# mbed92/soft-grip

Measured on AMD Instinct MI355X. Metric: env steps/sec (whole node) at batch=4096, higher is better.
Workload: dtype f64; 1 GPU; configs[2]: 4096 envs/GPU, softbox scene (nv=118), stiffness ~ U(300,1400), reference 200-step squeeze schedule from reset, 7 substeps per env step; 327 equality rows (composite neighbour equalities on: DESIGN.md 2, U2); volume tendon damper integrated explicitly; envs_per_gpu=4096, envs_flagged_bad=0

## Files before the change

### soft-grip_amd/csrc/sg_phase.hip

```cpp
#include "sg_work.h"

struct GenLds {
  StageRec2* stage;
  double* gas;
  double* gg;
  double* tmp;
  const double (*boxp)[3];
  const double (*boxm)[9];
  const ChainKin* K;
  const ChainLds2* cs;
  const double *qe, *ve, *asme, *we;
};

__device__ __forceinline__ void sg_gen_capsule(const SgPhaseArgs& a, const GenLds& L, int e, double* cp, double* cax) {
  const int N = a.nelem;
  auto EL = [&](int f, int k) { return a.elem[(size_t)f * N + k]; };
  const double dq = L.qe[e] - EL(SGE_QPOS0, e);
  cp[0] = EL(SGE_GX, e) + EL(SGE_AX, e) * dq; cp[1] = EL(SGE_GY, e) + EL(SGE_AY, e) * dq; cp[2] = EL(SGE_GZ, e) + EL(SGE_AZ, e) * dq;
  cax[0] = EL(SGE_CX, e); cax[1] = EL(SGE_CY, e); cax[2] = EL(SGE_CZ, e);
}

__device__ __noinline__ int sg_gen_phase(const SgPhaseArgs& a, const SgPlanHeader& H, const int env, const GenLds L, int* flags, int* touch) {
  const int lane = threadIdx.x, N = a.nelem;
  auto EL = [&](int f, int k) { return a.elem[(size_t)f * N + k]; };
// ... 656 lines not shown
          for (int r = 0; r < 3; r++) ro[(26 + r) * SG_SPW] = c.f[r];
          ((int*)(ro + 29 * SG_SPW))[0] = sl;
          }
        }
        const int nk = (ns0 > ns1 ? ns0 : ns1) - 32 * k;
        if (a.rowlayout && nk > 0) {
          const int nwb8 = (a.nenv + 7) / 8;
          const int li = lane & 31;
          auto X = [&](int sl_, int L) -> double2* {
            return (double2*)&Sm.stage[sl_ >> 4][32 * k] + ((sl_ & 15) * 8 + L);
          };
          __syncthreads();
          double2* const e0 = (double2*)&Sm.stage[li >> 4][32 * k] + ((li & 15) * 8 + 4 * half);
#pragma unroll
          for (int pr = 0; pr < SG_RK / 2; pr++) {
            e0[0] = fp[0][pr]; e0[1] = fp[1][pr]; e0[2] = fp[2][pr]; e0[3] = fp[3][pr];
            __syncthreads();
#pragma unroll
            for (int j = 0; j < 4; j++) {
              if (8 * j >= nk) break;
              const int e = j * 64 + lane, s_ = e >> 3, L = e & 7;
              if (s_ < nk) *(double2*)(W.crow + SG_ROW_INDEX(32 * k + s_, env >> 3, 2 * pr, 8 * (env & 7) + L, nwb8)) = *X(s_, L);
            }
            __syncthreads();
          }
        }
      }
      SG_T(5);
      double eqR[R], eqb[R], eqf[R];
      double tbp = 0, tjp = 0, tAp = 0;
#pragma unroll
      for (int r = 0; r < R; r++) {
        int e = r * 64 + lane;
        eqR[r] = 1; eqb[r] = 0; eqf[r] = 0;
        if (e < N) {
          double pos = qe[r] - EL(SGE_QPOS0, e), imp = impedance(H.eqj_solimp, pos, 0);
          eqR[r] = fmax(SG_MINVAL, (1 - imp) / imp * EL(SGE_INVW, e));
          double aref = -H.eqj_B * ve[r] - H.eqj_K * imp * pos;
          eqb[r] = asme[r] - aref;
          eqf[r] = -(we[r] - aref) / eqR[r];
          tbp += coef[r] * asme[r]; tjp += coef[r] * we[r]; tAp += coef[r] * coef[r] * invm[r];
        }
      }
      const int nnb = NB ? H.nnb : 0;
      constexpr int ND = NB ? 3 : 0;
      int nbe2[R][3], nbid[R][3];
      double nbc0[R][3];
      [[maybe_unused]] double nbff[R][3];
      [[maybe_unused]] double* const gnbf = W.nbf + (size_t)env * 3 * N;
#pragma unroll
      for (int r = 0; r < R; r++)
#pragma unroll
        for (int d = 0; d < 3; d++) { nbe2[r][d] = -1; nbid[r][d] = -1; nbc0[r][d] = 0; nbff[r][d] = 0; }
      if constexpr (NB) {
        const double im0 = 1.0 / (EL(SGE_MASS, 0) + EL(SGE_ARMATURE, 0));
        const SG_CONSTAS int* const cposc = (const SG_CONSTAS int*)a.cpos;
        const bool wantc = a.rowlayout && a.cst_rounds;
#pragma unroll
        for (int r = 0; r < R; r++) {
          const int e = r * 64 + lane;
          if (e < N) {
            double c4[4] = {0.0, 0.0, 0.0, 0.0};
            if (wantc) c4[0] = sg_div(im0, im0 + eqR[r]);
#pragma unroll
            for (int d = 0; d < 3; d++) {
              const int e2 = nbtabc[d * N + e];
              if (e2 >= 0) {
                const int id = nbtabc[(3 + d) * N + e];
                const double pos = (qe[r] - EL(SGE_QPOS0, e)) - (Sm.as[e2] - EL(SGE_QPOS0, e2)), imp = impedance(H.eqj_solimp, pos, 0);
                const double Rr = fmax(SG_MINVAL, (1 - imp) / imp * (EL(SGE_INVW, e) + EL(SGE_INVW, e2)));
                const double aref = -H.eqj_B * (ve[r] - Sm.ve[e2]) - H.eqj_K * imp * pos;
                const double bb = (asme[r] - Sm.asme[e2]) - aref, ff = -((we[r] - Sm.we[e2]) - aref) / Rr;
                nbe2[r][d] = e2; nbid[r][d] = id; nbc0[r][d] = ff * (0.5 * Rr * ff + bb);
                nbff[r][d] = ff; gnbf[id] = ff;
                W.nbb[(size_t)env * 3 * N + id] = bb; W.nbR[(size_t)env * 3 * N + id] = Rr;
                if (wantc) c4[1 + d] = sg_div(im0, 2.0 * im0 + Rr);
              }
            }
            if (wantc) {
              double* const dst = W.cst + SG_CST_INDEX(env >> 2, 0, 16 * (env & 3), a.cst_rounds) + cposc[e];
              *(double2*)dst = make_double2(c4[0], c4[1]);
              *(double2*)(dst + 2) = make_double2(c4[2], c4[3]);
            }
          }
        }
      }
      const double tpos = L0 - H.t0_L0, timp = impedance(H.eqt_solimp, tpos, 0), tR = fmax(SG_MINVAL, (1 - timp) / timp * H.eqt_invw);
      const double taref = -H.eqt_B * Ld - H.eqt_K * timp * tpos;
      const double tb = wave_sum2(tbp) - taref, tjar = wave_sum2(tjp) - taref, tA = wave_sum2(tAp) + tR;
      double tf = -tjar / tR;
      const int nmaxs = ns0 > ns1 ? ns0 : ns1;

      double aF[SG_CD];
      auto recompute_a = [&]() {
        __syncthreads();
#pragma unroll
        for (int r = 0; r < R; r++) {
          int e = r * 64 + lane;
          if (e < N) {
            double fe = eqf[r] + coef[r] * tf;
            if constexpr (NB) {
#pragma unroll
              for (int d = 0; d < 3; d++) if (nbid[r][d] >= 0) fe += nbff[r][d];
              double fin[3];
#pragma unroll
              for (int d = 0; d < 3; d++) { const int ii = nbtabc[(6 + d) * N + e]; fin[d] = ii >= 0 ? gnbf[ii] : 0.0; }
#pragma unroll
              for (int d = 0; d < 3; d++) fe -= fin[d];
            }
            double as_ = invm[r] * fe;
#pragma unroll
            for (int cb = 0; cb < SG_MAXCH * SG_CG; cb++) {
              const int u = Sm.eslot[e][cb], i0 = u & 0x3F, nst = u >> 6;
              if (nst >= 1) as_ += cval_at(cb / SG_CG, i0);
              if (nst >= 2) as_ += cval_at(cb / SG_CG, i0 + 1);
            }
            if constexpr (GEN)
              if (ngen) as_ += GL.gas[e];
            Sm.as[e] = as_;
          }
        }
        __syncthreads();
        double g[SG_CD] = {0, 0, 0, 0};
#pragma unroll
        for (int k = 0; k < CPL; k++)
#pragma unroll
          for (int d = 0; d < SG_CD; d++) g[d] += cg[k][d];
        if (is_chain_lane) {
          const int la = CS.lim_active;
#pragma unroll
          for (int k = 0; k < SG_MAXLIM; k++)
            if (la >> k & 1) g[k / 2] += CS.lim_sign[k] * CS.lim_f[k];
          if constexpr (GEN)
            if (ngen) {
#pragma unroll
              for (int d = 0; d < SG_CD; d++) g[d] += GL.gg[half * SG_CD + d];
            }
        }
#pragma unroll
        for (int d = 0; d < SG_CD; d++) {
          double x = g[d];
#pragma unroll
          for (int o = 16; o > 0; o >>= 1) x += __shfl_xor(x, o);
          g[d] = x;
        }
#pragma unroll
        for (int a2 = 0; a2 < SG_CD; a2++) {
          double s2 = 0;
#pragma unroll
          for (int b2 = 0; b2 < SG_CD; b2++) s2 += CS.Minv[4 * a2 + b2] * g[b2];
          aF[a2] = s2;
        }
        __syncthreads();
      };
      recompute_a();
      SG_T(6);
      {
        double cp = 0, tJap = 0;
#pragma unroll
        for (int r = 0; r < R; r++) {
          int e = r * 64 + lane;
          if (e < N) {
            double ae = Sm.as[e]; cp += eqf[r] * (0.5 * (ae + eqR[r] * eqf[r]) + eqb[r]); tJap += coef[r] * ae;
#pragma unroll
            for (int d = 0; d < ND; d++)
              if (nbid[r][d] >= 0) cp += 0.5 * nbff[r][d] * (ae - Sm.as[nbe2[r][d]]) + nbc0[r][d];
          }
        }
        double tJa = wave_sum2(tJap);
        if (lane == 0) cp += tf * (0.5 * (tJa + tR * tf) + tb);
        if (is_chain_lane) {
          const int la = CS.lim_active;
#pragma unroll
          for (int k = 0; k < SG_MAXLIM; k++)
            if (la >> k & 1) cp += CS.lim_f[k] * (0.5 * (CS.lim_sign[k] * aF[k / 2] + CS.lim_R[k] * CS.lim_f[k]) + CS.lim_b[k]);
        }
#pragma unroll
        for (int k = 0; k < CPL; k++)
          if ((lane & 31) + 32 * k < myn) {
            double as_ = csl_[k] >= 0 ? Sm.as[csl_[k]] : 0.0, ga = 0;
#pragma unroll
            for (int d = 0; d < SG_CD; d++) ga += cg[k][d] * aF[d];
            cp += 0.5 * (ga + cjsf[k] * as_) + ccost0[k];
          }
        [[maybe_unused]] double aF2[SG_MAXCH][SG_CD];
        if constexpr (GEN)
          if (ngen) {
#pragma unroll
            for (int d = 0; d < SG_CD; d++) {
              const double other = __shfl_xor(aF[d], 32);
              aF2[0][d] = high ? other : aF[d]; aF2[1][d] = high ? aF[d] : other;
            }
            cp += sg_gen_cost(a, env, ngen, aF2, Sm.as, 0);
          }
        double cost = wave_sum2(cp);
        if (cost > 0) {
          if constexpr (GEN)
            if (ngen) {
              sg_gen_cost(a, env, ngen, aF2, Sm.as, 1);
              for (int e = lane; e < N; e += 64) GL.gas[e] = 0.0;
              if (lane < SG_MAXCH * SG_CD) GL.gg[lane] = 0.0;
            }
#pragma unroll
          for (int r = 0; r < R; r++) {
            eqf[r] = 0;
#pragma unroll
            for (int d = 0; d < ND; d++) if (nbid[r][d] >= 0) { nbff[r][d] = 0.0; gnbf[nbid[r][d]] = 0.0; }
          }
          tf = 0;
          if (is_chain_lane) {
#pragma unroll
            for (int k = 0; k < SG_MAXLIM; k++) CS.lim_f[k] = 0;
          }
#pragma unroll
          for (int k = 0; k < CPL; k++) {
            int i = (lane & 31) + 32 * k;
            cjsf[k] = 0;
#pragma unroll
            for (int d = 0; d < SG_CD; d++) cg[k][d] = 0;
            if (i < myn) {
              cval_at(half, i) = 0.0;
              if (!a.rowlayout) {
              double* ro = W.crec + SG_REC_INDEX(i, env / SG_EPW, 0, 2 * (env % SG_EPW) + half, nwb);
#pragma unroll
              for (int r = 0; r < 3; r++) ro[(26 + r) * SG_SPW] = 0.0;
              }
              if (a.rowlayout) {
#pragma unroll
                for (int r = 0; r < 3; r++)
                  *(double2*)(W.crow + SG_ROW_INDEX(i, env >> 3, 6, 8 * (env & 7) + 4 * half + r, (a.nenv + 7) / 8)) = make_double2(0.0, 0.0);
              }
            }
          }
          __syncthreads();
          recompute_a();
        }
      }
      SG_T(7);
#pragma unroll
      for (int r = 0; r < R; r++) {
        int e = r * 64 + lane;
        if (e < N) {
          size_t o = (size_t)env * N + e;
          W.as[o] = Sm.as[e]; W.eqf[o] = eqf[r]; W.eqb[o] = eqb[r]; W.eqR[o] = eqR[r];
        }
      }
      if (is_chain_lane) {
        W.ns[st] = myn < SG_CAP ? myn : SG_CAP;
        W.lim_active[st] = CS.lim_active;
      }
      if (half < nchain) {
        static_assert(4 * SG_MAXLIM == 32, "one limit value per lane of a half");
        const int i = lane & 31;
        W.lim[(size_t)i * S + st] = (&CS.lim_sign[0])[i];
        if (i < SG_CD) W.saF[(size_t)i * S + st] = i == 0 ? aF[0] : (i == 1 ? aF[1] : (i == 2 ? aF[2] : aF[3]));
      }
      if (lane == 0) {
        W.envh[(size_t)0 * a.nenv + env] = tb; W.envh[(size_t)1 * a.nenv + env] = tR;
        W.envh[(size_t)2 * a.nenv + env] = tA; W.envh[(size_t)3 * a.nenv + env] = tf;
        W.shared[env] = shared_slider;
        W.pending[env] = 1;
        W.ncon[env] = ns0 + ns1 + ngen;
        W.gen[env] = ngen;
        W.nefc[env] = N + nnb + 1 + 3 * (ns0 + ns1 + ngen) + __popc(Sm.cs[0].lim_active) + (nchain > 1 ? __popc(Sm.cs[1].lim_active) : 0);
        W.touch[env] = touch;
      }
    }
  }

  SG_T(8);
  __syncthreads();
#pragma unroll
  for (int r = 0; r < R; r++) {
    int e = r * 64 + lane;
    if (e < N) { gq[e0 + e] = qe[r]; gv[e0 + e] = ve[r]; gw[e0 + e] = we[r]; }
  }
  if (lane == 0) {
    if (status | flags) atomicOr(&W.status[env], status | flags);
  }
  SG_T(9);
  SG_TEND();
}

#ifndef SG_X_PHASE_OCC
#define SG_X_PHASE_OCC 2
#endif
#ifndef SG_X_CPL
#define SG_X_CPL 2
#endif
template <int R, int CPL, bool NB, bool GEN = false>
__global__ __launch_bounds__(64, SG_X_PHASE_OCC) void sg_phase_kernel(SgPhaseArgs a) {
  if constexpr (GEN) {
    const int cnt = a.w.gen_count[0];
    a.do_finish = 0; a.do_reset = 0; a.sens = nullptr;
    for (int i = blockIdx.x; i < cnt && i < a.nenv; i += gridDim.x) {
      sg_phase_env<R, CPL, NB, true>(a, a.w.gen_list[i]);
      __syncthreads();
    }
  } else {
    sg_phase_env<R, CPL, NB, false>(a, blockIdx.x);
  }
}

__global__ __launch_bounds__(64) void sg_chain_kernel(SgPhaseArgs a) {
  const int lane = threadIdx.x, c = blockIdx.x & 1, env = (int)(blockIdx.x >> 1) * 64 + lane;
  if (blockIdx.x == 0 && lane == 0) a.w.gen_count[0] = 0;
  SG_T0();
  const SG_CONSTAS SgPlanHeader& H = *(const SG_CONSTAS SgPlanHeader*)a.H;
  const int nv = a.nv, nu = a.nu;
  const size_t S = 2 * (size_t)a.nenv;
  if (env >= a.nenv) return;
  const size_t st = 2 * (size_t)env + c;
  if (a.mask && !a.mask[env]) return;
  SgWork& W = a.w;
  if (a.first && c == 0) { W.status[env] = 0; if (!a.do_finish) W.pending[env] = 0; }
  if (c >= a.nchain) return;
  const int status = a.first ? 0 : W.status[env];
  const int pend = a.do_finish ? W.pending[env] : 0;
  const SgChain& C = H.chain[c];
  const double h = a.timestep;
  double* gq = a.qpos + (size_t)env * nv;
  double* gv = a.qvel + (size_t)env * nv;
  double* gw = a.warm + (size_t)env * nv;
  const double kenv = a.kenv[env];
  double q[SG_CD], v[SG_CD], w[SG_CD], kk[SG_CD], act = 0, ctrl = 0;
#pragma unroll
  for (int d = 0; d < SG_CD; d++) {
    int j = C.dof0 + d;
    if (a.do_reset) { q[d] = C.qpos0[d]; v[d] = 0; w[d] = 0; }
    else { q[d] = gq[j]; v[d] = gv[j]; w[d] = gw[j]; }
    kk[d] = a.kmask_jnt[j] ? kenv : C.stiffness[d];
  }
  if (C.has_act) {
    if (a.do_reset) a.ctrl[(size_t)env * nu + C.act_id] = 0;
    else { act = a.act[(size_t)env * nu + C.act_id]; ctrl = a.ctrl[(size_t)env * nu + C.act_id]; }
  }
  const double kten = C.has_ten ? (a.kmask_ten[C.ten_id] ? kenv : C.ten_k0) : 0.0;
  double* ch = W.chh + st * SG_CHW;
  bool bad_acc = false;
  if (status & (SG_FLAG_BADQPOS | SG_FLAG_BADQVEL | SG_FLAG_BADQACC)) return;

  SG_T(17);
  if (a.do_finish && pend) {
    double aF[SG_CD], qacc_c[SG_CD];
#pragma unroll
    for (int d = 0; d < SG_CD; d++) {
      aF[d] = W.saF[(size_t)d * S + st];
      qacc_c[d] = ch[SGH_QSM + d] + aF[d];
      if (isbad(qacc_c[d])) bad_acc = true;
    }
    ChainKin K;
    {
      double* kd = (double*)&K;
#pragma unroll
      for (int i = 0; i < 48; i++) kd[i] = ch[SGH_K + i];
    }
    if (a.sens) {
      ChainMotion Mo;
      chain_motion(C, K, v, qacc_c, H.gravity, Mo);
      double* so = a.sens + (size_t)env * a.sens_stride;
      for (int s = 0; s < C.nsite; s++) {
        int bi = C.s_body[s];
        double r3[3], sm[9], t[3], t2[3], acc[3], out[3], sbp[3], sbm[9], bw[3], bal[3];
        chain_body_pose(K, bi, sbp, sbm);
        mulmat3(r3, sbm, C.s_pos[s]);
        mulmat33(sm, sbm, C.s_mat[s]);
        for (int k = 0; k < 3; k++) { bw[k] = bi == 0 ? Mo.w[0][k] : Mo.w[SG_CB - 1][k]; bal[k] = bi == 0 ? Mo.al[0][k] : Mo.al[SG_CB - 1][k]; }
        if (C.s_gyro_adr[s] >= 0) {
          mulmatT3(out, sm, bw);
          for (int k = 0; k < 3; k++) so[C.s_gyro_adr[s] + k] = out[k];
        }
        if (C.s_acc_adr[s] >= 0) {
          for (int k = 0; k < 3; k++) acc[k] = bi == 0 ? Mo.a[0][k] : Mo.a[SG_CB - 1][k];
          cross3(t, bal, r3); addscl3(acc, t, 1);
          cross3(t, bw, r3); cross3(t2, bw, t); addscl3(acc, t2, 1);
          mulmatT3(out, sm, acc);
          for (int k = 0; k < 3; k++) so[C.s_acc_adr[s] + k] = out[k];
        }
      }
    }
    if (bad_acc) {
      atomicOr(&W.status[env], SG_FLAG_BADQACC);
    } else {
#pragma unroll
      for (int d = 0; d < SG_CD; d++) w[d] = qacc_c[d];
      if (a.finish_integrate) {
        bool damp = false;
#pragma unroll
        for (int d = 0; d < SG_CD; d++) damp |= C.damping[d] > 0;
        double qa[SG_CD];
        if (damp) {
          double MhB[16], MhBinv[16], rhs[SG_CD], Mm[16];
#pragma unroll
          for (int i = 0; i < 16; i++) { Mm[i] = ch[SGH_M + i]; MhB[i] = Mm[i]; }
#pragma unroll
          for (int d = 0; d < SG_CD; d++) MhB[5 * d] += h * C.damping[d];
          spd_inverse4(MhB, MhBinv);
#pragma unroll
          for (int a2 = 0; a2 < SG_CD; a2++) {
            double s2 = ch[SGH_QFRC + a2];
#pragma unroll
            for (int b2 = 0; b2 < SG_CD; b2++) s2 += Mm[4 * a2 + b2] * aF[b2];
            rhs[a2] = s2;
          }
#pragma unroll
          for (int a2 = 0; a2 < SG_CD; a2++) {
            double s2 = 0;
#pragma unroll
            for (int b2 = 0; b2 < SG_CD; b2++) s2 += MhBinv[4 * a2 + b2] * rhs[b2];
            qa[a2] = s2;
          }
        } else {
#pragma unroll
          for (int d = 0; d < SG_CD; d++) qa[d] = qacc_c[d];
        }
        act += h * ch[SGH_ACTDOT];
#pragma unroll
        for (int d = 0; d < SG_CD; d++) { v[d] += h * qa[d]; q[d] += h * v[d]; }
      }
    }
  }

  SG_T(18);
  if (a.do_begin && !bad_acc) {
    int bad = 0;
#pragma unroll
    for (int d = 0; d < SG_CD; d++) bad |= (isbad(q[d]) ? SG_FLAG_BADQPOS : 0) | (isbad(v[d]) ? SG_FLAG_BADQVEL : 0);
    if (bad) {
      atomicOr(&W.status[env], bad);
    } else {
      ChainKin K;
      ChainDyn D;
      chain_kinematics(C, q, K);
      SG_T(19);
      chain_dynamics(C, K, q, v, act, ctrl, kk, kten, H.gravity, D);
      SG_T(20);
      double rec[SG_CHW];
#pragma unroll
      for (int i = 0; i < SG_CHW; i++) rec[i] = 0.0;
#pragma unroll
      for (int d = 0; d < SG_CD; d++) { rec[SGH_QSM + d] = D.qacc_smooth[d]; rec[SGH_QFRC + d] = D.qfrc_smooth[d]; rec[SGH_V + d] = v[d]; rec[SGH_W + d] = w[d]; }
      rec[SGH_ACTDOT] = D.act_dot;
#pragma unroll
      for (int i = 0; i < 16; i++) { rec[SGH_M + i] = D.M[i]; rec[SGH_MINV + i] = D.Minv[i]; W.sMinv[(size_t)i * S + st] = D.Minv[i]; }
      {
        const double* kd = (const double*)&K;
#pragma unroll
        for (int i = 0; i < 48; i++) rec[SGH_K + i] = kd[i];
      }
#pragma unroll
      for (int g = 0; g < SG_CG; g++) {
        double t[3] = {0, 0, 0}, bp_[3] = {0, 0, 0}, bm_[9], bm2[9];
#pragma unroll
        for (int k = 0; k < 9; k++) bm2[k] = 0;
        if (g < C.ngeom) {
          chain_body_pose(K, C.g_body[g], bp_, bm_);
          mulmat3(t, bm_, C.g_pos[g]);
          mulmat33(bm2, bm_, C.g_mat[g]);
        }
#pragma unroll
        for (int k = 0; k < 3; k++) rec[SGH_BOX + 12 * g + k] = bp_[k] + t[k];
#pragma unroll
        for (int k = 0; k < 9; k++) rec[SGH_BOX + 12 * g + 3 + k] = bm2[k];
      }
      SG_T(21);
      LimitRows L;
      limits_build(C, q, v, D.qacc_smooth, w, L);
      rec[SGH_LIMACT] = (double)L.active;
#pragma unroll
      for (int k = 0; k < SG_MAXLIM; k++) { rec[SGH_LIMSIGN + k] = L.sign[k]; rec[SGH_LIMR + k] = L.R[k]; rec[SGH_LIMB + k] = L.b[k]; rec[SGH_LIMF + k] = L.f[k]; }
      static_assert(SG_CHW % 2 == 0 && SGH_LIMF + SG_MAXLIM <= SG_CHW, "hand-off record layout");
#pragma unroll
      for (int i = 0; i < (SGH_LIMF + SG_MAXLIM + 1) / 2; i++) ((double2*)ch)[i] = make_double2(rec[2 * i], rec[2 * i + 1]);
    }
  }
  SG_T(22);
#pragma unroll
  for (int d = 0; d < SG_CD; d++) { int j = C.dof0 + d; gq[j] = q[d]; gv[j] = v[d]; gw[j] = w[d]; }
  if (C.has_act) a.act[(size_t)env * nu + C.act_id] = act;
  SG_T(23);
  SG_TEND();
}


hipError_t sg_launch_chain(const SgPhaseArgs& p, int nenv, hipStream_t s) {
  hipLaunchKernelGGL(sg_chain_kernel, dim3(2 * ((nenv + 63) / 64)), dim3(64), 0, s, p);
  return hipGetLastError();
}
hipError_t sg_launch_phase(const SgPhaseArgs& p, int rounds, bool nb, bool genpass, int nenv, hipStream_t s) {
#define SG_PHASE(r)                                                                                   \
  if (nb) {                                                                                           \
    hipLaunchKernelGGL((sg_phase_kernel<r, SG_X_CPL, true>), dim3(nenv), dim3(64), 0, s, p);                 \
    if (genpass && p.do_begin) hipLaunchKernelGGL((sg_phase_kernel<r, 2, true, true>), dim3(nenv < SG_GEN_GRID ? nenv : SG_GEN_GRID), dim3(64), 0, s, p); \
  } else {                                                                                            \
    hipLaunchKernelGGL((sg_phase_kernel<r, SG_X_CPL, false>), dim3(nenv), dim3(64), 0, s, p);                \
    if (genpass && p.do_begin) hipLaunchKernelGGL((sg_phase_kernel<r, 2, false, true>), dim3(nenv < SG_GEN_GRID ? nenv : SG_GEN_GRID), dim3(64), 0, s, p); \
  }
  switch (rounds) {
    case 1: SG_PHASE(1); break;
    case 2: SG_PHASE(2); break;
    case 3: SG_PHASE(3); break;
    default: SG_PHASE(4); break;
  }
#undef SG_PHASE
  return hipGetLastError();
}
```

Baseline: 1.116 million env-steps/s.

## Stage chain params in LDS, widen chain workgroups, and stream hand-off record stores

The chain kernel now uses 256-thread workgroups and copies the per-chain SgChain struct into shared memory once per block, instead of every lane reading it from constant/global memory. The hand-off record is written as paired double2 stores right after each piece is computed, so the large rec[] register array goes away, and box poses are computed before dynamics. The kinematic copy in the finish path is moved inside the sensor branch so it only runs when sensors are used. The cost is a __syncthreads, shared memory use, and early-exit lanes that now have to stay through the barrier. An optional scalar-load warm-up path is added but is off by default.

```diff
diff --git a/soft-grip_amd/csrc/sg_phase.hip b/soft-grip_amd/csrc/sg_phase.hip
--- a/soft-grip_amd/csrc/sg_phase.hip
+++ b/soft-grip_amd/csrc/sg_phase.hip
@@ -982,27 +982,82 @@
   }
 }
 
-__global__ __launch_bounds__(64) void sg_chain_kernel(SgPhaseArgs a) {
-  const int lane = threadIdx.x, c = blockIdx.x & 1, env = (int)(blockIdx.x >> 1) * 64 + lane;
-  if (blockIdx.x == 0 && lane == 0) a.w.gen_count[0] = 0;
+#ifndef SG_X_CHAIN_WG
+#define SG_X_CHAIN_WG 256
+#endif
+#ifndef SG_X_CHAIN_LDS
+#define SG_X_CHAIN_LDS 1
+#endif
+#ifndef SG_X_CHAIN_WARM
+#define SG_X_CHAIN_WARM 0
+#endif
+#ifndef SG_X_CHAIN_STREAM
+#define SG_X_CHAIN_STREAM 1
+#endif
+#ifdef SG_SECTION_PROF
+#undef SG_TEND
+#define SG_TEND()                                                 \
+  do {                                                            \
+    if ((threadIdx.x & 63) == 0)                                  \
+      for (int k_ = 0; k_ < 26; k_++)                             \
+        if (t_acc_[k_]) atomicAdd(&a.w.secprof[k_], t_acc_[k_]);  \
+  } while (0)
+#endif
+__device__ __forceinline__ void sg_ch_store2(double* ch, int i, double x, double y) { ((double2*)ch)[i >> 1] = make_double2(x, y); }
+
+__global__ __launch_bounds__(SG_X_CHAIN_WG) void sg_chain_kernel(SgPhaseArgs a) {
+  const int tid = threadIdx.x, c = blockIdx.x & 1, env = (int)(blockIdx.x >> 1) * SG_X_CHAIN_WG + tid;
+  if (blockIdx.x == 0 && tid == 0) a.w.gen_count[0] = 0;
   SG_T0();
   const SG_CONSTAS SgPlanHeader& H = *(const SG_CONSTAS SgPlanHeader*)a.H;
   const int nv = a.nv, nu = a.nu;
   const size_t S = 2 * (size_t)a.nenv;
-  if (env >= a.nenv) return;
+  const bool have = env < a.nenv && !(a.mask && !a.mask[env]);
+  SgWork& W = a.w;
+  if (have && a.first && c == 0) { W.status[env] = 0; if (!a.do_finish) W.pending[env] = 0; }
+  const bool live = have && c < a.nchain;
+  const int status = live && !a.first ? W.status[env] : 0;
+  const int pend = live && a.do_finish ? W.pending[env] : 0;
+  const double kenv = live ? a.kenv[env] : 0.0;
+#if SG_X_CHAIN_LDS
+  __shared__ __attribute__((aligned(16))) SgChain Cs;
+  {
+    static_assert(sizeof(SgChain) % 16 == 0 && offsetof(SgPlanHeader, chain) % 16 == 0, "SgChain is copied in 16-byte pieces");
+    constexpr int NP = (int)(sizeof(SgChain) / 16);
+    const SG_CONSTAS double2* src = (const SG_CONSTAS double2*)&H.chain[c];
+    double2* dst = (double2*)&Cs;
+#pragma unroll
+    for (int k = 0; k < (NP + SG_X_CHAIN_WG - 1) / SG_X_CHAIN_WG; k++) {
+      const int i = k * SG_X_CHAIN_WG + tid;
+      if (i < NP) dst[i] = src[i];
+    }
+  }
+  __syncthreads();
+  const SgChain& C = Cs;
+#else
+#if SG_X_CHAIN_WARM
+  {
+    typedef int sg_v16i __attribute__((ext_vector_type(16)));
+    static_assert(sizeof(SgChain) == 29 * 64, "the warm-up below requests 29 pieces of 64 bytes");
+    const SG_CONSTAS char* wp = (const SG_CONSTAS char*)&H.chain[c];
+    sg_v16i wt;
+#define SG_WL(o) "s_load_dwordx16 %0, %1, " #o "\n\t"
+    asm volatile(SG_WL(0x0) SG_WL(0x40) SG_WL(0x80) SG_WL(0xc0) SG_WL(0x100) SG_WL(0x140) SG_WL(0x180) SG_WL(0x1c0) SG_WL(0x200) SG_WL(0x240)
+                 SG_WL(0x280) SG_WL(0x2c0) SG_WL(0x300) SG_WL(0x340) SG_WL(0x380) SG_WL(0x3c0) SG_WL(0x400) SG_WL(0x440) SG_WL(0x480) SG_WL(0x4c0)
+                 SG_WL(0x500) SG_WL(0x540) SG_WL(0x580) SG_WL(0x5c0) SG_WL(0x600) SG_WL(0x640) SG_WL(0x680) SG_WL(0x6c0) SG_WL(0x700)
+                 "s_waitcnt lgkmcnt(0)"
+                 : "=&s"(wt) : "s"(wp) : "memory");
+#undef SG_WL
+  }
+#endif
+  const SgChain& C = H.chain[c];
+#endif
+  if (!live) return;
   const size_t st = 2 * (size_t)env + c;
-  if (a.mask && !a.mask[env]) return;
-  SgWork& W = a.w;
-  if (a.first && c == 0) { W.status[env] = 0; if (!a.do_finish) W.pending[env] = 0; }
-  if (c >= a.nchain) return;
-  const int status = a.first ? 0 : W.status[env];
-  const int pend = a.do_finish ? W.pending[env] : 0;
-  const SgChain& C = H.chain[c];
   const double h = a.timestep;
   double* gq = a.qpos + (size_t)env * nv;
   double* gv = a.qvel + (size_t)env * nv;
   double* gw = a.warm + (size_t)env * nv;
-  const double kenv = a.kenv[env];
   double q[SG_CD], v[SG_CD], w[SG_CD], kk[SG_CD], act = 0, ctrl = 0;
 #pragma unroll
   for (int d = 0; d < SG_CD; d++) {
@@ -1029,13 +1084,13 @@
       qacc_c[d] = ch[SGH_QSM + d] + aF[d];
       if (isbad(qacc_c[d])) bad_acc = true;
     }
-    ChainKin K;
-    {
-      double* kd = (double*)&K;
-#pragma unroll
-      for (int i = 0; i < 48; i++) kd[i] = ch[SGH_K + i];
-    }
     if (a.sens) {
+      ChainKin K;
+      {
+        double* kd = (double*)&K;
+#pragma unroll
+        for (int i = 0; i < 48; i++) kd[i] = ch[SGH_K + i];
+      }
       ChainMotion Mo;
       chain_motion(C, K, v, qacc_c, H.gravity, Mo);
       double* so = a.sens + (size_t)env * a.sens_stride;
@@ -1113,6 +1168,68 @@
       ChainDyn D;
       chain_kinematics(C, q, K);
       SG_T(19);
+#if SG_X_CHAIN_STREAM
+      static_assert(SG_CHW % 2 == 0 && SGH_LIMF + SG_MAXLIM <= SG_CHW, "hand-off record layout");
+      static_assert(SGH_K % 2 == 1 && SGH_M % 2 == 1 && SGH_MINV % 2 == 1 && SGH_V % 2 == 1 && SGH_W == SGH_V + 4 && SGH_BOX == SGH_W + 4 &&
+                    SGH_LIMACT == SGH_BOX + 24 && SGH_LIMSIGN % 2 == 0 && SGH_ACTDOT == SGH_M - 1 && SGH_K == SGH_M + 16 &&
+                    SGH_MINV == SGH_K + 48 && SGH_V == SGH_MINV + 16, "the pairs below follow this layout");
+      const double* const kd = (const double*)&K;
+#pragma unroll
+      for (int i = 1; i < 47; i += 2) sg_ch_store2(ch, SGH_K + i, kd[i], kd[i + 1]);
+      sg_ch_store2(ch, SGH_V + 1, v[1], v[2]);
+      sg_ch_store2(ch, SGH_V + 3, v[3], w[0]);
+      sg_ch_store2(ch, SGH_W + 1, w[1], w[2]);
+      double box0 = 0, box23 = 0;
+      {
+        double bx[12 * SG_CG];
+#pragma unroll
+        for (int g = 0; g < SG_CG; g++) {
+          double t[3] = {0, 0, 0}, bp_[3] = {0, 0, 0}, bm_[9], bm2[9];
+#pragma unroll
+          for (int k = 0; k < 9; k++) bm2[k] = 0;
+          if (g < C.ngeom) {
+            chain_body_pose(K, C.g_body[g], bp_, bm_);
+            mulmat3(t, bm_, C.g_pos[g]);
+            mulmat33(bm2, bm_, C.g_mat[g]);
+          }
+#pragma unroll
+          for (int k = 0; k < 3; k++) bx[12 * g + k] = bp_[k] + t[k];
+#pragma unroll
+          for (int k = 0; k < 9; k++) bx[12 * g + 3 + k] = bm2[k];
+        }
+#pragma unroll
+        for (int i = 1; i < 12 * SG_CG - 1; i += 2) sg_ch_store2(ch, SGH_BOX + i, bx[i], bx[i + 1]);
+        box0 = bx[0]; box23 = bx[12 * SG_CG - 1];
+      }
+      SG_T(21);
+      chain_dynamics(C, K, q, v, act, ctrl, kk, kten, H.gravity, D);
+      SG_T(20);
+      sg_ch_store2(ch, SGH_QSM, D.qacc_smooth[0], D.qacc_smooth[1]);
+      sg_ch_store2(ch, SGH_QSM + 2, D.qacc_smooth[2], D.qacc_smooth[3]);
+      sg_ch_store2(ch, SGH_QFRC, D.qfrc_smooth[0], D.qfrc_smooth[1]);
+      sg_ch_store2(ch, SGH_QFRC + 2, D.qfrc_smooth[2], D.qfrc_smooth[3]);
+      sg_ch_store2(ch, SGH_ACTDOT, D.act_dot, D.M[0]);
+#pragma unroll
+      for (int i = 1; i < 15; i += 2) sg_ch_store2(ch, SGH_M + i, D.M[i], D.M[i + 1]);
+      sg_ch_store2(ch, SGH_M + 15, D.M[15], kd[0]);
+      sg_ch_store2(ch, SGH_K + 47, kd[47], D.Minv[0]);
+#pragma unroll
+      for (int i = 1; i < 15; i += 2) sg_ch_store2(ch, SGH_MINV + i, D.Minv[i], D.Minv[i + 1]);
+      sg_ch_store2(ch, SGH_MINV + 15, D.Minv[15], v[0]);
+      sg_ch_store2(ch, SGH_W + 3, w[3], box0);
+#pragma unroll
+      for (int i = 0; i < 16; i++) W.sMinv[(size_t)i * S + st] = D.Minv[i];
+      LimitRows L;
+      limits_build(C, q, v, D.qacc_smooth, w, L);
+      sg_ch_store2(ch, SGH_LIMACT - 1, box23, (double)L.active);
+#pragma unroll
+      for (int k = 0; k < SG_MAXLIM; k += 2) {
+        sg_ch_store2(ch, SGH_LIMSIGN + k, L.sign[k], L.sign[k + 1]);
+        sg_ch_store2(ch, SGH_LIMR + k, L.R[k], L.R[k + 1]);
+        sg_ch_store2(ch, SGH_LIMB + k, L.b[k], L.b[k + 1]);
+        sg_ch_store2(ch, SGH_LIMF + k, L.f[k], L.f[k + 1]);
+      }
+#else
       chain_dynamics(C, K, q, v, act, ctrl, kk, kten, H.gravity, D);
       SG_T(20);
       double rec[SG_CHW];
@@ -1152,6 +1269,7 @@
       static_assert(SG_CHW % 2 == 0 && SGH_LIMF + SG_MAXLIM <= SG_CHW, "hand-off record layout");
 #pragma unroll
       for (int i = 0; i < (SGH_LIMF + SG_MAXLIM + 1) / 2; i++) ((double2*)ch)[i] = make_double2(rec[2 * i], rec[2 * i + 1]);
+#endif
     }
   }
   SG_T(22);
@@ -1164,7 +1282,7 @@
 
 
 hipError_t sg_launch_chain(const SgPhaseArgs& p, int nenv, hipStream_t s) {
-  hipLaunchKernelGGL(sg_chain_kernel, dim3(2 * ((nenv + 63) / 64)), dim3(64), 0, s, p);
+  hipLaunchKernelGGL(sg_chain_kernel, dim3(2 * ((nenv + SG_X_CHAIN_WG - 1) / SG_X_CHAIN_WG)), dim3(SG_X_CHAIN_WG), 0, s, p);
   return hipGetLastError();
 }
 hipError_t sg_launch_phase(const SgPhaseArgs& p, int rounds, bool nb, bool genpass, int nenv, hipStream_t s) {
```

Result: slower. 1.100 million env-steps/s (-1.4%).
